# myshell-ai/OpenVoice

Measured on NVIDIA H100. Metric: audio_seconds_per_second, higher is better.
Workload: dtype f32 (3xFP16 split-precision tensor-core convs with fp32 accumulation, fp32 FFMA elsewhere)

## Files before the change

openvoice_b200/csrc/ovc_tcconv.cuh:

```cuda
#pragma once
#include "ovc_conv.cuh"
#include "ovc_tc.cuh"
#include "ovc_tcpack.h"

namespace ovc {

struct TcConvArgs {
  const float* x; long long x_bs;
  const uint16_t* w;
  const float* bias; long long bias_bs;
  float* y; long long y_bs; int y_ld;
  const float* r;
  float* s; long long s_bs;
  int epi;
  int split; int first;
  const long long* lens; int tmax; int mul;
  const long long* lens_x; int has_lens_x;
  int Cin; int Ntot; int K; int DIL;
  float slope; float scale; int accumulate;
  int passes;
  const uint16_t* w2; const float* bias2;
};

__device__ __forceinline__ void pdl_launch_dependents() { asm volatile("griddepcontrol.launch_dependents;" ::: "memory"); }
__device__ __forceinline__ void pdl_wait() { asm volatile("griddepcontrol.wait;" ::: "memory"); }

__device__ __forceinline__ void mbar_arrive(uint64_t* bar) {
  asm volatile("mbarrier.arrive.shared::cta.b64 _, [%0];" ::"r"(smem_u32(bar)) : "memory");
}
__device__ __forceinline__ void named_bar_sync(int id, int threads) {
  asm volatile("bar.sync %0, %1;" ::"r"(id), "r"(threads) : "memory");
}

template <int TN>
__device__ __forceinline__ void tc_epilogue(const TcConvArgs& a, const float (&d)[TN], int b, int t0, int n0, int lim, int row_a) {
  const int csub = (threadIdx.x & 3) * 2;
  float* yb = a.y + (size_t)b * a.y_bs;
  const float* rb = a.r ? a.r + (size_t)b * a.y_bs : nullptr;
  float* sb = a.s ? a.s + (size_t)b * a.s_bs : nullptr;
  const float* bias = a.bias + (size_t)b * a.bias_bs;
  const bool two = a.passes == 3;
  const int ta = t0 + row_a, tb = ta + 8;
  const bool oka = ta < lim, okb = tb < lim;
#pragma unroll
  for (int c0 = 0; c0 < TN; c0 += 32) {
    float v[16];
#pragma unroll
    for (int i = 0; i < 16; ++i) v[i] = two ? fmaf(d[TN / 2 + c0 / 2 + i], tc::kLoInv, d[c0 / 2 + i]) : d[c0 / 2 + i];
#pragma unroll
    for (int g = 0; g < 4; ++g) {
      const float2 bq = __ldg(reinterpret_cast<const float2*>(bias + n0 + c0 + 8 * g + csub));
      v[4 * g] += bq.x; v[4 * g + 1] += bq.y; v[4 * g + 2] += bq.x; v[4 * g + 3] += bq.y;
    }
    if (a.epi == 0) {
      float* ypa = yb + (size_t)ta * a.y_ld + n0 + c0 + csub;
      float* ypb = yb + (size_t)tb * a.y_ld + n0 + c0 + csub;
      const float* rpa = rb ? rb + (size_t)ta * a.y_ld + n0 + c0 + csub : nullptr;
      const float* rpb = rb ? rb + (size_t)tb * a.y_ld + n0 + c0 + csub : nullptr;
#pragma unroll
      for (int g = 0; g < 4; ++g) {
        float2 oa = make_float2(v[4 * g], v[4 * g + 1]), ob = make_float2(v[4 * g + 2], v[4 * g + 3]);
        if (rb) {
          const float2 qa = oka ? *reinterpret_cast<const float2*>(rpa + 8 * g) : make_float2(0.f, 0.f);
          const float2 qb = okb ? *reinterpret_cast<const float2*>(rpb + 8 * g) : make_float2(0.f, 0.f);
          oa.x += qa.x; oa.y += qa.y; ob.x += qb.x; ob.y += qb.y;
        }
        if (a.accumulate) {
          const float2 ya = oka ? *reinterpret_cast<const float2*>(ypa + 8 * g) : make_float2(0.f, 0.f);
          const float2 yc = okb ? *reinterpret_cast<const float2*>(ypb + 8 * g) : make_float2(0.f, 0.f);
          oa.x = ya.x + oa.x; oa.y = ya.y + oa.y;
          ob.x = yc.x + ob.x; ob.y = yc.y + ob.y;
        }
        if (a.scale != 1.f) { oa.x *= a.scale; oa.y *= a.scale; ob.x *= a.scale; ob.y *= a.scale; }
        if (oka) *reinterpret_cast<float2*>(ypa + 8 * g) = oa;
        if (okb) *reinterpret_cast<float2*>(ypb + 8 * g) = ob;
      }
    } else if (a.epi == 1) {
      float* ypa = yb + (size_t)ta * a.y_ld + ((n0 + c0) >> 1) + csub;
      float* ypb = yb + (size_t)tb * a.y_ld + ((n0 + c0) >> 1) + csub;
#pragma unroll
      for (int g = 0; g < 2; ++g) {
        const float2 oa = make_float2(tanhf(v[4 * g]) * sigmoidf_acc(v[4 * (g + 2)]),
                                      tanhf(v[4 * g + 1]) * sigmoidf_acc(v[4 * (g + 2) + 1]));
        const float2 ob = make_float2(tanhf(v[4 * g + 2]) * sigmoidf_acc(v[4 * (g + 2) + 2]),
                                      tanhf(v[4 * g + 3]) * sigmoidf_acc(v[4 * (g + 2) + 3]));
        if (oka) *reinterpret_cast<float2*>(ypa + 8 * g) = oa;
        if (okb) *reinterpret_cast<float2*>(ypb + 8 * g) = ob;
      }
    } else {
      const int col = n0 + c0;
      const bool to_x = col < a.split;
      const bool add = to_x || !a.first;
      float* dst = (to_x ? yb + col : sb + (col - a.split)) + csub;
#pragma unroll
      for (int g = 0; g < 4; ++g) {
        float2 oa = make_float2(v[4 * g], v[4 * g + 1]), ob = make_float2(v[4 * g + 2], v[4 * g + 3]);
        if (add) {
          const float2 qa = oka ? *reinterpret_cast<const float2*>(dst + (size_t)ta * a.y_ld + 8 * g) : make_float2(0.f, 0.f);
          const float2 qb = okb ? *reinterpret_cast<const float2*>(dst + (size_t)tb * a.y_ld + 8 * g) : make_float2(0.f, 0.f);
          oa = make_float2(qa.x + oa.x, qa.y + oa.y);
          ob = make_float2(qb.x + ob.x, qb.y + ob.y);
        }
        if (oka) *reinterpret_cast<float2*>(dst + (size_t)ta * a.y_ld + 8 * g) = oa;
        if (okb) *reinterpret_cast<float2*>(dst + (size_t)tb * a.y_ld + 8 * g) = ob;
      }
    }
  }
}

template <int TN>
__device__ __forceinline__ void tc_mma_step(float (&d)[TN], uint64_t a_hi, uint64_t a_lo, uint64_t b, bool three, bool first) {
  float (&lo)[TN / 2] = *reinterpret_cast<float(*)[TN / 2]>(&d[TN / 2]);
  float (&hi)[TN / 2] = *reinterpret_cast<float(*)[TN / 2]>(&d[0]);
  tc::Wgmma<TN>::mma(hi, a_hi, b, first ? 0 : 1);
  if (three) {
    tc::Wgmma<TN>::mma(lo, a_hi, b + TN, first ? 0 : 1);
    tc::Wgmma<TN>::mma(lo, a_lo, b, 1);
  }
}

constexpr int TCN_THREADS = 384;
constexpr int TCN_NCT = 96;

template <int TN, bool PAIR>
struct TcnCfg {
  static_assert(!PAIR || TN == 32 || TN == 64 || TN == 128, "conv pairs: C = 32, 64 or 128");
  static constexpr int KCH = 32, NKC = KCH / 8;
  static constexpr int ROWS = 194;
  static constexpr int ROWS2 = TCN_ROWS2;
  static constexpr int NABUF = 2;
  static constexpr int RING = tc_ring_slots(TN, PAIR);
  static constexpr int SLOT_BYTES = 2 * 2 * TN * 16;
  static constexpr int A_BUF_BYTES = 2 * NKC * ROWS * 16;
  static constexpr int A2_BYTES = PAIR ? 2 * (TN / 8) * ROWS2 * 16 : 0;
  static constexpr size_t SMEM_BYTES = 1024 + NABUF * A_BUF_BYTES + A2_BYTES + RING * SLOT_BYTES;
  static_assert(SMEM_BYTES <= 232448, "shared memory budget");
  static_assert((2 * NABUF + 2 * RING) * 8 <= 1024, "barrier area");
};

constexpr int TCN_PROD_REGS = 56, TCN_MMA_REGS = 224;

template <int TN, bool PAIR>
__global__ void __launch_bounds__(TCN_THREADS, 1) tcconv_kernel(const TcConvArgs a, int n_tt, int total) {
  using Cfg = TcnCfg<TN, PAIR>;
  constexpr int ROWS = Cfg::ROWS, ROWS2 = Cfg::ROWS2, NABUF = Cfg::NABUF, RING = Cfg::RING, NKC = Cfg::NKC;
  extern __shared__ __align__(128) unsigned char smem_raw[];
  uint64_t* bars = reinterpret_cast<uint64_t*>(smem_raw);
  uint64_t *a_full = bars, *a_empty = bars + NABUF, *b_full = a_empty + NABUF, *b_empty = b_full + RING;
  unsigned char* abuf = smem_raw + 1024;
  unsigned char* a2buf = abuf + NABUF * Cfg::A_BUF_BYTES;
  unsigned char* bring = a2buf + Cfg::A2_BYTES;

  const int tid = threadIdx.x, lane = tid & 31;
  const int warp = __shfl_sync(0xffffffffu, tid >> 5, 0);
  const int H1 = (a.K - 1) / 2 * a.DIL;
  const int H2 = PAIR ? (a.K - 1) / 2 : 0;
  const int R = 128 - 2 * H2;
  const int rows8 = (128 + 2 * H1 + 7) & ~7;
  const int nq = a.Cin / Cfg::KCH;
  const int n_slots = (a.Cin / 16) * a.K;
  const int n_w = PAIR ? 2 * n_slots : n_slots;
  const bool resident = n_w <= RING;
  if (H1 > TCN_HMAX || (PAIR && 128 + 2 * H2 > ROWS2)) __trap();
  constexpr uint32_t BYTES = Cfg::SLOT_BYTES;

  if (tid == 0) {
    for (int i = 0; i < NABUF; ++i) { mbar_init(&a_full[i], TCN_NCT); mbar_init(&a_empty[i], 2); }
    for (int i = 0; i < RING; ++i) { mbar_init(&b_full[i], 1); mbar_init(&b_empty[i], 2); }
    fence_mbar_init();
  }
  if (PAIR) {
    for (int i = tid; i < Cfg::A2_BYTES / 16; i += TCN_THREADS) reinterpret_cast<uint4*>(a2buf)[i] = make_uint4(0u, 0u, 0u, 0u);
    asm volatile("fence.proxy.async.shared::cta;" ::: "memory");
  }
  __syncthreads();
  pdl_launch_dependents();
  if (warp != 0) pdl_wait();

#define TCN_FOR_TILES                                                                                   \
  for (int tile = blockIdx.x; tile < total; tile += gridDim.x) {                                        \
    const int b = tile / n_tt, t0 = (tile % n_tt) * R;                                                  \
    const int lim = (a.lens ? (int)min((long long)a.tmax, a.lens[b]) : a.tmax) * a.mul;                 \
    const int lim_x = a.has_lens_x ? (int)min((long long)a.tmax, a.lens_x[b]) * a.mul : lim;            \
    (void)lim_x;                                                                                        \
    if (t0 >= lim) continue;

  if (warp < 4) {
    tc::regs_dealloc<TCN_PROD_REGS>();
    if (warp == 0) {
      if (lane == 0) {
        const unsigned char* wt = reinterpret_cast<const unsigned char*>(a.w) + (size_t)blockIdx.y * n_slots * BYTES;
        if (resident) {
          for (int it = 0; it < n_w; ++it) {
            const unsigned char* src = it < n_slots ? wt + (size_t)it * BYTES
                                                    : reinterpret_cast<const unsigned char*>(a.w2) + (size_t)(it - n_slots) * BYTES;
            mbar_expect_tx(&b_full[it], BYTES);
            tma_bulk_g2s(bring + it * BYTES, src, BYTES, &b_full[it]);
          }
          for (int it = 0; it < n_w; ++it) mbar_wait(&b_full[it], 0u);
        } else {
          int slot = 0;
          uint32_t phase = 1;
          TCN_FOR_TILES
            (void)b;
            for (int it = 0; it < n_w; ++it) {
              const unsigned char* src = it < n_slots ? wt + (size_t)it * BYTES
                                                      : reinterpret_cast<const unsigned char*>(a.w2) + (size_t)(it - n_slots) * BYTES;
              mbar_wait(&b_empty[slot], phase);
              mbar_expect_tx(&b_full[slot], BYTES);
              tma_bulk_g2s(bring + slot * BYTES, src, BYTES, &b_full[slot]);
              if (++slot == RING) { slot = 0; phase ^= 1; }
            }
          }
        }
      }
    } else {
      const int pt = tid - 32;
      const int items = rows8 * NKC;
      int buf = 0;
      uint32_t ephase = 1;
      TCN_FOR_TILES
        const float* xb = a.x + (size_t)b * a.x_bs;
        const int r0 = t0 - H2 - H1;
        for (int q = 0; q < nq; ++q) {
          mbar_wait(&a_empty[buf], ephase);
          unsigned char* ah = abuf + buf * Cfg::A_BUF_BYTES;
          unsigned char* al = ah + NKC * ROWS * 16;
          constexpr int PB = 2;
          for (int i0 = pt; i0 < items; i0 += TCN_NCT * PB) {
            float4 v0[PB], v1[PB];
#pragma unroll
            for (int u = 0; u < PB; ++u) {
              const int i = i0 + TCN_NCT * u;
              const int row = i >> 2, kc = i & 3;
              const int t = r0 + row;
              v0[u] = make_float4(0.f, 0.f, 0.f, 0.f);
              v1[u] = v0[u];
              if (i < items && t >= 0 && t < lim_x) {
                const float4* src = reinterpret_cast<const float4*>(xb + (size_t)t * a.Cin + q * Cfg::KCH + kc * 8);
                v0[u] = src[0];
                v1[u] = src[1];
              }
            }
#pragma unroll
            for (int u = 0; u < PB; ++u) {
              const int i = i0 + TCN_NCT * u;
              if (i >= items) break;
              const int row = i >> 2, kc = i & 3;
              uint4 hi, lo;
              tc::split_f16x8(v0[u], v1[u], a.slope, hi, lo);
              *reinterpret_cast<uint4*>(ah + (kc * ROWS + row) * 16) = hi;
              *reinterpret_cast<uint4*>(al + (kc * ROWS + row) * 16) = lo;
            }
          }
          asm volatile("fence.proxy.async.shared::cta;" ::: "memory");
          mbar_arrive(&a_full[buf]);
          if (++buf == NABUF) { buf = 0; ephase ^= 1; }
        }
      }
    }
  } else {
    tc::regs_alloc<TCN_MMA_REGS>();
    const int wg = (warp >> 2) - 1;
    const bool leader = (tid & 127) == 0;
    const int row_a = 64 * wg + 16 * (warp & 3) + (lane >> 2);
    constexpr uint32_t LBO_A = ROWS * 16, LBO_A2 = ROWS2 * 16, LBO_B = 2 * TN * 16, SBO = 128;
    constexpr uint32_t A_LO16 = (NKC * ROWS * 16) >> 4, A2_LO16 = ((TN / 8) * ROWS2 * 16) >> 4, SLOT16 = BYTES >> 4;
    const uint64_t a_proto = tc::make_desc(0, LBO_A, SBO), b_proto = tc::make_desc(0, LBO_B, SBO);
    const uint64_t b_ring = b_proto + (tc::smem_addr(bring) >> 4);
    const bool three = a.passes == 3;
    float d[TN];
#pragma unroll
    for (int i = 0; i < TN; ++i) d[i] = 0.f;
    if (resident)
      for (int it = 0; it < n_w; ++it) mbar_wait(&b_full[it], 0u);
    int slot = 0, buf = 0;
    uint32_t bphase = 0, aphase = 0;
    TCN_FOR_TILES
      (void)lim_x;
      bool first = true;
      if (resident) slot = 0;
      for (int q = 0; q < nq; ++q) {
        mbar_wait(&a_full[buf], aphase);
        tc::fence_regs(d);
        tc::wgmma_fence();
        int prev = -1;
        for (int j = 0; j < 2; ++j) {
          uint64_t a_cur = a_proto + ((tc::smem_addr(abuf + buf * Cfg::A_BUF_BYTES) + 64 * wg * 16 + 2 * j * LBO_A) >> 4);
          for (int tap = 0; tap < a.K; ++tap) {
            if (!resident) mbar_wait(&b_full[slot], bphase);
            tc_mma_step<TN>(d, a_cur, a_cur + A_LO16, b_ring + (uint32_t)slot * SLOT16, three, first);
            tc::wgmma_commit();
            if (!resident) {
              tc::wgmma_wait<1>();
              if (leader && prev >= 0) mbar_arrive(&b_empty[prev]);
              prev = slot;
            }
            first = false;
            a_cur += a.DIL;
            if (++slot == RING) { slot = 0; bphase ^= 1; }
          }
        }
        tc::wgmma_wait<0>();
        tc::fence_regs(d);
        if (leader) {
          if (prev >= 0) mbar_arrive(&b_empty[prev]);
          mbar_arrive(&a_empty[buf]);
        }
        if (++buf == NABUF) { buf = 0; aphase ^= 1; }
      }
      if constexpr (!PAIR) {
        tc_epilogue<TN>(a, d, b, t0, blockIdx.y * TN, lim, row_a);
      } else {
        named_bar_sync(1, 256);
        unsigned char* a2h = a2buf;
        unsigned char* a2l = a2buf + (TN / 8) * ROWS2 * 16;
        const int ta = t0 - H2 + row_a, tb = ta + 8;
        const bool oka = ta >= 0 && ta < lim, okb = tb >= 0 && tb < lim;
        const int csub = (lane & 3) * 2;
#pragma unroll
        for (int g = 0; g < TN / 8; ++g) {
          const float2 bq = __ldg(reinterpret_cast<const float2*>(a.bias + 8 * g + csub));
          float x[4];
#pragma unroll
          for (int i = 0; i < 4; ++i) x[i] = (three ? fmaf(d[TN / 2 + 4 * g + i], tc::kLoInv, d[4 * g + i]) : d[4 * g + i]) + ((i & 1) ? bq.y : bq.x);
          x[0] = oka ? fmaxf(x[0], x[0] * a.slope) : 0.f;
          x[1] = oka ? fmaxf(x[1], x[1] * a.slope) : 0.f;
          x[2] = okb ? fmaxf(x[2], x[2] * a.slope) : 0.f;
          x[3] = okb ? fmaxf(x[3], x[3] * a.slope) : 0.f;
          const __half2 ha = __floats2half2_rn(x[0], x[1]), hb = __floats2half2_rn(x[2], x[3]);
          const float2 fa = __half22float2(ha), fb = __half22float2(hb);
          const __half2 la = __floats2half2_rn((x[0] - fa.x) * tc::kLoScale, (x[1] - fa.y) * tc::kLoScale);
          const __half2 lb = __floats2half2_rn((x[2] - fb.x) * tc::kLoScale, (x[3] - fb.y) * tc::kLoScale);
          const int oa = (g * ROWS2 + row_a) * 16 + (lane & 3) * 4, ob = oa + 8 * 16;
          *reinterpret_cast<__half2*>(a2h + oa) = ha;
          *reinterpret_cast<__half2*>(a2h + ob) = hb;
          *reinterpret_cast<__half2*>(a2l + oa) = la;
          *reinterpret_cast<__half2*>(a2l + ob) = lb;
        }
        asm volatile("fence.proxy.async.shared::cta;" ::: "memory");
        named_bar_sync(2, 256);
        const uint64_t a2_proto = tc::make_desc(0, LBO_A2, SBO);
        tc::fence_regs(d);
        tc::wgmma_fence();
        bool first2 = true;
        int prev = -1;
        for (int kk = 0; kk < TN / 16; ++kk) {
          uint64_t a_cur = a2_proto + ((tc::smem_addr(a2buf) + 64 * wg * 16 + 2 * kk * LBO_A2) >> 4);
          for (int tap = 0; tap < a.K; ++tap) {
            if (resident) {
              tc_mma_step<TN>(d, a_cur, a_cur + A2_LO16, b_ring + (uint32_t)(n_slots + kk * a.K + tap) * SLOT16, three, first2);
            } else {
              mbar_wait(&b_full[slot], bphase);
              tc_mma_step<TN>(d, a_cur, a_cur + A2_LO16, b_ring + (uint32_t)slot * SLOT16, three, first2);
              tc::wgmma_commit();
              tc::wgmma_wait<1>();
              if (leader && prev >= 0) mbar_arrive(&b_empty[prev]);
              prev = slot;
              if (++slot == RING) { slot = 0; bphase ^= 1; }
            }
            first2 = false;
            a_cur += 1;
          }
        }
        tc::wgmma_commit();
        tc::wgmma_wait<0>();
        tc::fence_regs(d);
        if (leader && prev >= 0) mbar_arrive(&b_empty[prev]);
        TcConvArgs e = a;
        e.y_ld = TN; e.r = a.x; e.bias = a.bias2; e.bias_bs = 0; e.epi = 0;
        tc_epilogue<TN>(e, d, b, t0, 0, min(lim, t0 + R), row_a);
      }
    }
  }
#undef TCN_FOR_TILES
}

template <int C>
__global__ void __launch_bounds__(256) conv_post_cl_kernel(const float* __restrict__ x, long long x_bs,
                                                           const float* __restrict__ w, float* __restrict__ y,
                                                           long long y_bs, int y_len, const long long* lens, int tmax,
                                                           int mul) {
  constexpr int TB = 256, ROWS = TB + 6, LD = ROWS + 3;
  __shared__ float ws[7][C];
  __shared__ float xs[C][LD];
  for (int i = threadIdx.x; i < C * 7; i += blockDim.x) ws[i % 7][i / 7] = w[i];
  const int b = blockIdx.y;
  const int lim = (lens ? (int)min((long long)tmax, lens[b]) : tmax) * mul;
  const int t0 = blockIdx.x * TB;
  const float* xb = x + (size_t)b * x_bs;
  for (int idx = threadIdx.x; idx < ROWS * (C / 4); idx += blockDim.x) {
    const int row = idx / (C / 4), q = idx % (C / 4);
    const int tt = t0 - 3 + row;
    float4 v = make_float4(0.f, 0.f, 0.f, 0.f);
    if (tt >= 0 && tt < lim) v = *reinterpret_cast<const float4*>(xb + (size_t)tt * C + 4 * q);
    xs[4 * q + 0][row] = v.x > 0.f ? v.x : 0.01f * v.x;
    xs[4 * q + 1][row] = v.y > 0.f ? v.y : 0.01f * v.y;
    xs[4 * q + 2][row] = v.z > 0.f ? v.z : 0.01f * v.z;
    xs[4 * q + 3][row] = v.w > 0.f ? v.w : 0.01f * v.w;
  }
  __syncthreads();
  const int t = t0 + threadIdx.x;
  if (t >= y_len) return;
  float acc = 0.f;
  if (t < lim) {
#pragma unroll
    for (int k = 0; k < 7; ++k)
#pragma unroll 8
      for (int ci = 0; ci < C; ++ci) acc = fmaf(ws[k][ci], xs[ci][threadIdx.x + k], acc);
    acc = tanhf(acc);
  }
  y[(size_t)b * y_bs + t] = acc;
}

__global__ void __launch_bounds__(256) transpose_kernel(const float* __restrict__ src, float* __restrict__ dst, int rows,
                                                        int cols, long long bs) {
  __shared__ float tile[32][33];
  const float* s = src + (size_t)blockIdx.z * bs;
  float* d = dst + (size_t)blockIdx.z * bs;
  const int c0 = blockIdx.x * 32, r0 = blockIdx.y * 32;
  const int tx = threadIdx.x & 31, ty = threadIdx.x >> 5;
  for (int i = ty; i < 32; i += 8) {
    const int r = r0 + i, c = c0 + tx;
    tile[i][tx] = (r < rows && c < cols) ? s[(size_t)r * cols + c] : 0.f;
  }
  __syncthreads();
  for (int i = ty; i < 32; i += 8) {
    const int c = c0 + i, r = r0 + tx;
    if (r < rows && c < cols) d[(size_t)c * rows + r] = tile[tx][i];
  }
}

}
```

openvoice_b200/csrc/ovc_tcpack.h:

```cpp
#pragma once
#include <cuda_fp16.h>
#include <stddef.h>
#include <stdint.h>

#include <algorithm>

namespace ovc {

constexpr int TCN_HMAX = 25;
constexpr int TCN_ROWS2 = 146;

constexpr int tc_ring_slots(int TN, bool pair) {
  return pair ? (TN == 32 ? 44 : TN == 64 ? 24 : 12) : (TN == 32 ? 22 : 12);
}

struct TcGeom {
  int Cin = 0, Ntot = 0, K = 0, DIL = 1, TN = 0;
};

inline int tc_tile_n(int Ntot, int Cin, int K, int DIL) {
  if (Ntot <= 0 || Cin <= 0 || K <= 0 || DIL <= 0) return 0;
  if (Ntot % 32 || Cin % 32 || (K - 1) / 2 * DIL > TCN_HMAX) return 0;
  return Ntot % 128 == 0 ? 128 : (Ntot % 64 == 0 ? 64 : 32);
}

inline size_t tc_slot_halfs(int TN) { return (size_t)2 * 2 * TN * 8; }
inline size_t tc_packed_halfs(int Ntot, int Cin, int K, int TN) {
  return TN ? (size_t)(Ntot / TN) * (Cin / 16) * K * tc_slot_halfs(TN) : 0;
}
inline size_t tc_packed_index(int Cin, int K, int TN, int n, int ci, int tap, int part) {
  const int nt = n / TN, k16 = ci / 16, kc = (ci % 16) / 8, e = ci % 8;
  const size_t slot = ((size_t)nt * (Cin / 16) + k16) * K + tap;
  return slot * tc_slot_halfs(TN) + ((size_t)(kc * 2 + part) * TN + n % TN) * 8 + e;
}

inline void tc_split(float w, uint16_t& hi, uint16_t& lo) {
  const __half h = __float2half_rn(w);
  const __half l = __float2half_rn((w - __half2float(h)) * 2048.f);
  hi = __half_as_ushort(h);
  lo = __half_as_ushort(l);
}

template <class WF>
inline void tc_pack_weights(uint16_t* dst, int Ntot, int Cin, int K, int TN, WF wfun) {
  for (int nt = 0; nt < Ntot / TN; ++nt)
    for (int k16 = 0; k16 < Cin / 16; ++k16)
      for (int tap = 0; tap < K; ++tap) {
        uint16_t* sl = dst + (((size_t)nt * (Cin / 16) + k16) * K + tap) * tc_slot_halfs(TN);
        for (int kc = 0; kc < 2; ++kc)
          for (int n = 0; n < TN; ++n)
            for (int e = 0; e < 8; ++e) {
              uint16_t hi, lo;
              tc_split(wfun(nt * TN + n, k16 * 16 + kc * 8 + e, tap), hi, lo);
              sl[((kc * 2 + 0) * TN + n) * 8 + e] = hi;
              sl[((kc * 2 + 1) * TN + n) * 8 + e] = lo;
            }
      }
}

template <class RAW>
inline float tc_ups_weight(RAW raw, int s, int kk, int cout, int row, int ci, int tap) {
  const int pad = (kk - s) / 2;
  const int ph = row / cout, co = row % cout;
  const int kidx = s * (1 - tap) + ph + pad;
  return (kidx >= 0 && kidx < kk) ? raw(ci, co, kidx) : 0.f;
}

inline bool tc_pair_fits(const TcGeom& T1, const TcGeom& T2) {
  if (!(T1.TN == 32 || T1.TN == 64)) return false;
  const int ring = tc_ring_slots(T1.TN, true);
  return T1.Ntot == T1.TN && T1.Cin == T1.TN && T2.Ntot == T1.TN && T2.Cin == T1.TN && T2.TN == T1.TN && T2.K == T1.K &&
         T2.DIL == 1 && (T1.K - 1) / 2 * T1.DIL <= TCN_HMAX && 2 * (T1.Cin / 16) * T1.K <= ring && T1.K <= 5;
}

inline bool tc_pair_fuses(const TcGeom& T1, const TcGeom& T2) {
  if (!(T1.TN == 32 || T1.TN == 64 || T1.TN == 128)) return false;
  return T1.Ntot == T1.TN && T1.Cin == T1.TN && T2.Ntot == T1.TN && T2.Cin == T1.TN && T2.TN == T1.TN && T2.K == T1.K &&
         T2.DIL == 1 && (T1.K - 1) / 2 * T1.DIL <= TCN_HMAX && 128 + 2 * ((T2.K - 1) / 2) <= TCN_ROWS2;
}

struct TcGrid {
  int n_tt = 0, total = 0, grid_x = 0, ncol = 0;
};
inline TcGrid tc_grid(int t_len, int B, int Ntot, int TN, int sm_count, int grid_div) {
  TcGrid g;
  g.n_tt = (t_len + 127) / 128;
  g.total = g.n_tt * B;
  g.ncol = Ntot / TN;
  const int per_col = std::max(1, sm_count / g.ncol / std::max(1, grid_div));
  g.grid_x = std::min(g.total, per_col);
  return g;
}
inline TcGrid tc_pair_grid(int t_len, int B, int K, int sm_count) {
  TcGrid g;
  const int R = 128 - (K - 1);
  g.n_tt = (t_len + R - 1) / R;
  g.total = g.n_tt * B;
  g.ncol = 1;
  g.grid_x = std::min(g.total, sm_count);
  return g;
}

}
```

Before: 2225.

## Prefetch epilogue operands and next-tile input rows into L2, double-buffer epilogue loads

```diff
diff --git a/openvoice_b200/csrc/ovc_tcconv.cuh b/openvoice_b200/csrc/ovc_tcconv.cuh
--- a/openvoice_b200/csrc/ovc_tcconv.cuh
+++ b/openvoice_b200/csrc/ovc_tcconv.cuh
@@ -42,6 +42,42 @@
   const bool two = a.passes == 3;
   const int ta = t0 + row_a, tb = ta + 8;
   const bool oka = ta < lim, okb = tb < lim;
+  auto rs_dst = [&](int c0) { const int col = n0 + c0; return (col < a.split ? yb + col : sb + (col - a.split)) + csub; };
+  auto rs_add = [&](int c0) { return n0 + c0 < a.split || !a.first; };
+  auto load = [&](int c0, float2 (&p)[8], float2 (&q)[8]) {
+    const float2 z = make_float2(0.f, 0.f);
+#pragma unroll
+    for (int i = 0; i < 8; ++i) p[i] = q[i] = z;
+    if (a.epi == 0) {
+      if (rb) {
+        const float* rpa = rb + (size_t)ta * a.y_ld + n0 + c0 + csub;
+        const float* rpb = rb + (size_t)tb * a.y_ld + n0 + c0 + csub;
+#pragma unroll
+        for (int g = 0; g < 4; ++g) {
+          if (oka) p[2 * g] = *reinterpret_cast<const float2*>(rpa + 8 * g);
+          if (okb) p[2 * g + 1] = *reinterpret_cast<const float2*>(rpb + 8 * g);
+        }
+      }
+      if (a.accumulate) {
+        const float* ypa = yb + (size_t)ta * a.y_ld + n0 + c0 + csub;
+        const float* ypb = yb + (size_t)tb * a.y_ld + n0 + c0 + csub;
+#pragma unroll
+        for (int g = 0; g < 4; ++g) {
+          if (oka) q[2 * g] = *reinterpret_cast<const float2*>(ypa + 8 * g);
+          if (okb) q[2 * g + 1] = *reinterpret_cast<const float2*>(ypb + 8 * g);
+        }
+      }
+    } else if (a.epi == 2 && rs_add(c0)) {
+      const float* dst = rs_dst(c0);
+#pragma unroll
+      for (int g = 0; g < 4; ++g) {
+        if (oka) p[2 * g] = *reinterpret_cast<const float2*>(dst + (size_t)ta * a.y_ld + 8 * g);
+        if (okb) p[2 * g + 1] = *reinterpret_cast<const float2*>(dst + (size_t)tb * a.y_ld + 8 * g);
+      }
+    }
+  };
+  float2 p[8], q[8];
+  load(0, p, q);
 #pragma unroll
   for (int c0 = 0; c0 < TN; c0 += 32) {
     float v[16];
@@ -52,22 +88,20 @@
       const float2 bq = __ldg(reinterpret_cast<const float2*>(bias + n0 + c0 + 8 * g + csub));
       v[4 * g] += bq.x; v[4 * g + 1] += bq.y; v[4 * g + 2] += bq.x; v[4 * g + 3] += bq.y;
     }
+    float2 pn[8], qn[8];
+    if (c0 + 32 < TN) load(c0 + 32, pn, qn);
     if (a.epi == 0) {
       float* ypa = yb + (size_t)ta * a.y_ld + n0 + c0 + csub;
       float* ypb = yb + (size_t)tb * a.y_ld + n0 + c0 + csub;
-      const float* rpa = rb ? rb + (size_t)ta * a.y_ld + n0 + c0 + csub : nullptr;
-      const float* rpb = rb ? rb + (size_t)tb * a.y_ld + n0 + c0 + csub : nullptr;
 #pragma unroll
       for (int g = 0; g < 4; ++g) {
         float2 oa = make_float2(v[4 * g], v[4 * g + 1]), ob = make_float2(v[4 * g + 2], v[4 * g + 3]);
         if (rb) {
-          const float2 qa = oka ? *reinterpret_cast<const float2*>(rpa + 8 * g) : make_float2(0.f, 0.f);
-          const float2 qb = okb ? *reinterpret_cast<const float2*>(rpb + 8 * g) : make_float2(0.f, 0.f);
+          const float2 qa = p[2 * g], qb = p[2 * g + 1];
           oa.x += qa.x; oa.y += qa.y; ob.x += qb.x; ob.y += qb.y;
         }
         if (a.accumulate) {
-          const float2 ya = oka ? *reinterpret_cast<const float2*>(ypa + 8 * g) : make_float2(0.f, 0.f);
-          const float2 yc = okb ? *reinterpret_cast<const float2*>(ypb + 8 * g) : make_float2(0.f, 0.f);
+          const float2 ya = q[2 * g], yc = q[2 * g + 1];
           oa.x = ya.x + oa.x; oa.y = ya.y + oa.y;
           ob.x = yc.x + ob.x; ob.y = yc.y + ob.y;
         }
@@ -88,16 +122,13 @@
         if (okb) *reinterpret_cast<float2*>(ypb + 8 * g) = ob;
       }
     } else {
-      const int col = n0 + c0;
-      const bool to_x = col < a.split;
-      const bool add = to_x || !a.first;
-      float* dst = (to_x ? yb + col : sb + (col - a.split)) + csub;
+      const bool add = rs_add(c0);
+      float* dst = rs_dst(c0);
 #pragma unroll
       for (int g = 0; g < 4; ++g) {
         float2 oa = make_float2(v[4 * g], v[4 * g + 1]), ob = make_float2(v[4 * g + 2], v[4 * g + 3]);
         if (add) {
-          const float2 qa = oka ? *reinterpret_cast<const float2*>(dst + (size_t)ta * a.y_ld + 8 * g) : make_float2(0.f, 0.f);
-          const float2 qb = okb ? *reinterpret_cast<const float2*>(dst + (size_t)tb * a.y_ld + 8 * g) : make_float2(0.f, 0.f);
+          const float2 qa = p[2 * g], qb = p[2 * g + 1];
           oa = make_float2(qa.x + oa.x, qa.y + oa.y);
           ob = make_float2(qb.x + ob.x, qb.y + ob.y);
         }
@@ -105,7 +136,17 @@
         if (okb) *reinterpret_cast<float2*>(dst + (size_t)tb * a.y_ld + 8 * g) = ob;
       }
     }
-  }
+    if (c0 + 32 < TN) {
+#pragma unroll
+      for (int i = 0; i < 8; ++i) { p[i] = pn[i]; q[i] = qn[i]; }
+    }
+  }
+}
+
+__device__ __forceinline__ void prefetch_rows_l2(const float* base, TcSpan s, int row_floats) {
+  if (s.hi <= s.lo) return;
+  const float* p = base + (size_t)s.lo * row_floats;
+  asm volatile("cp.async.bulk.prefetch.L2.global [%0], %1;" ::"l"(p), "r"((uint32_t)(s.hi - s.lo) * row_floats * 4u) : "memory");
 }
 
 template <int TN>
@@ -177,11 +218,15 @@
   pdl_launch_dependents();
   if (warp != 0) pdl_wait();
 
+  auto limits = [&](int b) {
+    const int lim = (a.lens ? (int)min((long long)a.tmax, a.lens[b]) : a.tmax) * a.mul;
+    return make_int2(lim, a.has_lens_x ? (int)min((long long)a.tmax, a.lens_x[b]) * a.mul : lim);
+  };
 #define TCN_FOR_TILES                                                                                   \
   for (int tile = blockIdx.x; tile < total; tile += gridDim.x) {                                        \
     const int b = tile / n_tt, t0 = (tile % n_tt) * R;                                                  \
-    const int lim = (a.lens ? (int)min((long long)a.tmax, a.lens[b]) : a.tmax) * a.mul;                 \
-    const int lim_x = a.has_lens_x ? (int)min((long long)a.tmax, a.lens_x[b]) * a.mul : lim;            \
+    const int2 lims = limits(b);                                                                        \
+    const int lim = lims.x, lim_x = lims.y;                                                             \
     (void)lim_x;                                                                                        \
     if (t0 >= lim) continue;
 
@@ -220,6 +265,14 @@
       int buf = 0;
       uint32_t ephase = 1;
       TCN_FOR_TILES
+        if (pt == 0) {
+          const int nt = tile + gridDim.x;
+          if (nt < total) {
+            const int nb = nt / n_tt, nt0 = (nt % n_tt) * R;
+            const int2 nl = limits(nb);
+            if (nt0 < nl.x) prefetch_rows_l2(a.x + (size_t)nb * a.x_bs, tc_row_span(nt0 - H2 - H1, rows8, nl.y), a.Cin);
+          }
+        }
         const float* xb = a.x + (size_t)b * a.x_bs;
         const int r0 = t0 - H2 - H1;
         for (int q = 0; q < nq; ++q) {
@@ -263,7 +316,7 @@
     tc::regs_alloc<TCN_MMA_REGS>();
     const int wg = (warp >> 2) - 1;
     const bool leader = (tid & 127) == 0;
-    const int row_a = 64 * wg + 16 * (warp & 3) + (lane >> 2);
+    auto row_a = [] { return (int)(16 * ((threadIdx.x - 128) >> 5) + ((threadIdx.x & 31) >> 2)); };
     constexpr uint32_t LBO_A = ROWS * 16, LBO_A2 = ROWS2 * 16, LBO_B = 2 * TN * 16, SBO = 128;
     constexpr uint32_t A_LO16 = (NKC * ROWS * 16) >> 4, A2_LO16 = ((TN / 8) * ROWS2 * 16) >> 4, SLOT16 = BYTES >> 4;
     const uint64_t a_proto = tc::make_desc(0, LBO_A, SBO), b_proto = tc::make_desc(0, LBO_B, SBO);
@@ -278,6 +331,18 @@
     uint32_t bphase = 0, aphase = 0;
     TCN_FOR_TILES
       (void)lim_x;
+      if (leader && wg == 0) {
+        const TcSpan s = tc_row_span(t0, R, lim);
+        const int ld = PAIR ? TN : a.y_ld;
+        if (a.epi == 0) {
+          if (a.accumulate) prefetch_rows_l2(a.y + (size_t)b * a.y_bs, s, ld);
+          if (!PAIR && a.r) prefetch_rows_l2(a.r + (size_t)b * a.y_bs, s, ld);
+        } else if (a.epi == 2) {
+          const int n0 = blockIdx.y * TN;
+          if (n0 < a.split) prefetch_rows_l2(a.y + (size_t)b * a.y_bs, s, ld);
+          if (n0 + TN > a.split && !a.first) prefetch_rows_l2(a.s + (size_t)b * a.s_bs, s, ld);
+        }
+      }
       bool first = true;
       if (resident) slot = 0;
       for (int q = 0; q < nq; ++q) {
@@ -310,12 +375,12 @@
         if (++buf == NABUF) { buf = 0; aphase ^= 1; }
       }
       if constexpr (!PAIR) {
-        tc_epilogue<TN>(a, d, b, t0, blockIdx.y * TN, lim, row_a);
+        tc_epilogue<TN>(a, d, b, t0, blockIdx.y * TN, lim, row_a());
       } else {
         named_bar_sync(1, 256);
         unsigned char* a2h = a2buf;
         unsigned char* a2l = a2buf + (TN / 8) * ROWS2 * 16;
-        const int ta = t0 - H2 + row_a, tb = ta + 8;
+        const int ra = row_a(), ta = t0 - H2 + ra, tb = ta + 8;
         const bool oka = ta >= 0 && ta < lim, okb = tb >= 0 && tb < lim;
         const int csub = (lane & 3) * 2;
 #pragma unroll
@@ -332,7 +397,7 @@
           const float2 fa = __half22float2(ha), fb = __half22float2(hb);
           const __half2 la = __floats2half2_rn((x[0] - fa.x) * tc::kLoScale, (x[1] - fa.y) * tc::kLoScale);
           const __half2 lb = __floats2half2_rn((x[2] - fb.x) * tc::kLoScale, (x[3] - fb.y) * tc::kLoScale);
-          const int oa = (g * ROWS2 + row_a) * 16 + (lane & 3) * 4, ob = oa + 8 * 16;
+          const int oa = (g * ROWS2 + ra) * 16 + (lane & 3) * 4, ob = oa + 8 * 16;
           *reinterpret_cast<__half2*>(a2h + oa) = ha;
           *reinterpret_cast<__half2*>(a2h + ob) = hb;
           *reinterpret_cast<__half2*>(a2l + oa) = la;
@@ -369,7 +434,7 @@
         if (leader && prev >= 0) mbar_arrive(&b_empty[prev]);
         TcConvArgs e = a;
         e.y_ld = TN; e.r = a.x; e.bias = a.bias2; e.bias_bs = 0; e.epi = 0;
-        tc_epilogue<TN>(e, d, b, t0, 0, min(lim, t0 + R), row_a);
+        tc_epilogue<TN>(e, d, b, t0, 0, min(lim, t0 + R), row_a());
       }
     }
   }
diff --git a/openvoice_b200/csrc/ovc_tcpack.h b/openvoice_b200/csrc/ovc_tcpack.h
--- a/openvoice_b200/csrc/ovc_tcpack.h
+++ b/openvoice_b200/csrc/ovc_tcpack.h
@@ -4,6 +4,12 @@
 #include <stdint.h>
 
 #include <algorithm>
+
+#if defined(__CUDACC__)
+#define OVC_TC_HD __host__ __device__ __forceinline__
+#else
+#define OVC_TC_HD inline
+#endif
 
 namespace ovc {
 
@@ -101,4 +107,13 @@
   return g;
 }
 
+struct TcSpan {
+  int lo, hi;
+};
+OVC_TC_HD TcSpan tc_row_span(int first, int count, int lim) {
+  const int lo = first > 0 ? first : 0;
+  const int hi = first + count < lim ? first + count : lim;
+  return TcSpan{lo, hi > lo ? hi : lo};
 }
+
+}
```

New measurement: 2269, median of 6. 2.0% higher.
